# Frikallo/parakeet.cpp

Measured on NVIDIA H100. Metric: audio-seconds/sec (RTFx) tdt-ctc-110m 10s clips, higher is better.
Workload: dtype bf16x3

## Files before the change

### parakeet.cpp_b200/csrc/gemm_tc.cu

```cuda
#include <cuda.h>

#include "kernels.h"
#include "tc_prims.cuh"

namespace pk {
namespace {

using namespace tc;

constexpr int TC_THREADS = 384;
constexpr int CONSUMER_WARPS = 8;

template <int BN, int NPASS, bool LN = false>
struct TcCfg {
    static constexpr int A_BYTES = BM * BK * 2;
    static constexpr int W_BYTES = BN * BK * 2;
    static constexpr int PLANES = (NPASS == 3) ? 2 : 1;
    static constexpr int STAGE_BYTES = PLANES * (A_BYTES + W_BYTES);
    static constexpr int STAT_BYTES = LN ? 4 * BM * 4 * 4 : 0;
    static constexpr int AVAIL = 227 * 1024 - STAT_BYTES - 1024 - 256;
    static constexpr int STAGES = AVAIL / STAGE_BYTES > 8 ? 8 : AVAIL / STAGE_BYTES;
    static constexpr size_t SMEM = (size_t)STAGES * STAGE_BYTES + STAT_BYTES + 1024  + 256 ;
    static_assert(STAGES >= 2, "pipeline depth");
};

constexpr int LN_CL = 4;

template <int BN, int EK>
__device__ __forceinline__ void epilogue_regs(const float (&d)[BN / 2], const EpiParams &epi_param, int row0, int n0, int M, int N, int lane) {
    const EpiParams epi = epi_param;
    const int q = lane & 3;
    const int row = row0 + (lane >> 2) + ((q & 1) ? 8 : 0);
    const bool vec_ok = ((epi.ldo & 3) == 0) && ((N & 3) == 0);
    constexpr int G = 4;
#pragma unroll
    for (int j0 = 0; j0 < BN / 8; j0 += G) {
        float4 b[G], r[G];
#pragma unroll
        for (int g = 0; g < G; ++g) {
            const int col = n0 + 8 * (j0 + g) + 4 * (q >> 1);
            b[g] = r[g] = make_float4(0.f, 0.f, 0.f, 0.f);
            if (row < M && vec_ok && col + 4 <= N) {
                if (epi.bias) b[g] = __ldg(reinterpret_cast<const float4 *>(epi.bias + col));
                if (EK == EPI_RESID_F32) r[g] = *reinterpret_cast<const float4 *>(epi.resid + (size_t)row * epi.ldo + col);
            }
        }
#pragma unroll
        for (int g = 0; g < G; ++g) {
            const int j = j0 + g;
            const float s0 = (q & 1) ? d[4 * j] : d[4 * j + 2], s1 = (q & 1) ? d[4 * j + 1] : d[4 * j + 3];
            const float r0 = __shfl_xor_sync(0xffffffffu, s0, 1), r1 = __shfl_xor_sync(0xffffffffu, s1, 1);
            if (row >= M) continue;
            float4 v = (q & 1) ? make_float4(r0, r1, d[4 * j + 2], d[4 * j + 3]) : make_float4(d[4 * j], d[4 * j + 1], r0, r1);
            const int col = n0 + 8 * j + 4 * (q >> 1);
            if (vec_ok && col + 4 <= N) epi_store<EK>(epi, row, col, epi_math<EK>(v, b[g], r[g], epi.alpha));
            else epilogue4(epi_param, row, col, N, v);
        }
    }
}

template <int N>
__device__ __forceinline__ void fence_operands(float (&d)[N]) {
#pragma unroll
    for (int i = 0; i < N; ++i) asm volatile("" : "+f"(d[i])::"memory");
}

__device__ __forceinline__ float cluster_row_sum(float part, float *buf, int lrow, bool writer, uint32_t rank) {
    if (writer) {
        const uint32_t a = smem_u32(buf + lrow * LN_CL + rank);
#pragma unroll
        for (uint32_t r = 0; r < (uint32_t)LN_CL; ++r) st_cluster_f32(mapa_rank(a, r), part);
    }
    cluster_sync();
    const float4 v = *reinterpret_cast<const float4 *>(buf + lrow * LN_CL);
    return ((v.x + v.y) + v.z) + v.w;
}

__device__ __forceinline__ void epilogue_ln(const float (&d)[64], const LnEpi &ep, int row0, int lrow0, int n0, int M, int N, int lane,
                                            float *stat, uint32_t rank) {
    const int q = lane & 3;
    const int row = row0 + (lane >> 2) + ((q & 1) ? 8 : 0), lrow = lrow0 + (lane >> 2) + ((q & 1) ? 8 : 0);
    const bool writer = (q >> 1) == 0, live = row < M;
    float x[64];
#pragma unroll
    for (int j = 0; j < 16; ++j) {
        const float s0 = (q & 1) ? d[4 * j] : d[4 * j + 2], s1 = (q & 1) ? d[4 * j + 1] : d[4 * j + 3];
        const float r0 = __shfl_xor_sync(0xffffffffu, s0, 1), r1 = __shfl_xor_sync(0xffffffffu, s1, 1);
        const float4 v = (q & 1) ? make_float4(r0, r1, d[4 * j + 2], d[4 * j + 3]) : make_float4(d[4 * j], d[4 * j + 1], r0, r1);
        const int col = n0 + 8 * j + 4 * (q >> 1);
        float4 b = make_float4(0.f, 0.f, 0.f, 0.f), r = b;
        if (ep.bias) b = __ldg(reinterpret_cast<const float4 *>(ep.bias + col));
        if (ep.resid && live) r = *reinterpret_cast<const float4 *>(ep.resid + (size_t)row * N + col);
        x[4 * j] = r.x + ep.alpha * (v.x + b.x);
        x[4 * j + 1] = r.y + ep.alpha * (v.y + b.y);
        x[4 * j + 2] = r.z + ep.alpha * (v.z + b.z);
        x[4 * j + 3] = r.w + ep.alpha * (v.w + b.w);
    }
    auto store_f32 = [&]() {
        if (!live || !ep.out_f32) return;
#pragma unroll
        for (int j = 0; j < 16; ++j)
            *reinterpret_cast<float4 *>(ep.out_f32 + (size_t)row * N + n0 + 8 * j + 4 * (q >> 1)) =
                make_float4(x[4 * j], x[4 * j + 1], x[4 * j + 2], x[4 * j + 3]);
    };
    auto layernorm = [&](const float *w, const float *bb, float *buf) {
        float s = 0.f;
#pragma unroll
        for (int i = 0; i < 64; ++i) s += x[i];
        s += __shfl_xor_sync(0xffffffffu, s, 2);
        const float mean = cluster_row_sum(s, buf, lrow, writer, rank) / (float)N;
        float c = 0.f;
#pragma unroll
        for (int i = 0; i < 64; ++i) c += (x[i] - mean) * (x[i] - mean);
        c += __shfl_xor_sync(0xffffffffu, c, 2);
        const float rstd = rsqrtf(cluster_row_sum(c, buf + BM * LN_CL, lrow, writer, rank) / (float)N + ep.eps);
#pragma unroll
        for (int j = 0; j < 16; ++j) {
            const int col = n0 + 8 * j + 4 * (q >> 1);
            const float4 g = __ldg(reinterpret_cast<const float4 *>(w + col)), o = __ldg(reinterpret_cast<const float4 *>(bb + col));
            x[4 * j] = (x[4 * j] - mean) * rstd * g.x + o.x;
            x[4 * j + 1] = (x[4 * j + 1] - mean) * rstd * g.y + o.y;
            x[4 * j + 2] = (x[4 * j + 2] - mean) * rstd * g.z + o.z;
            x[4 * j + 3] = (x[4 * j + 3] - mean) * rstd * g.w + o.w;
        }
    };
    if (!ep.out_ln1) store_f32();
    layernorm(ep.ln1_w, ep.ln1_b, stat);
    if (ep.out_ln1) store_f32();
    if (ep.ln2_w) layernorm(ep.ln2_w, ep.ln2_b, stat + 2 * BM * LN_CL);
    if (live) {
#pragma unroll
        for (int j = 0; j < 16; ++j)
            store_act4(ep.planes, (size_t)row * N + n0 + 8 * j + 4 * (q >> 1), make_float4(x[4 * j], x[4 * j + 1], x[4 * j + 2], x[4 * j + 3]));
    }
}

template <int BN, int NPASS, int EK, int CL, bool MC, bool LN>
__device__ __forceinline__ void gemm_tc_body(const CUtensorMap &tmA_hi, const CUtensorMap &tmA_lo, const CUtensorMap &tmW_hi,
                                             const CUtensorMap &tmW_lo, int M, int N, int K, const EpiParams &epi, const LnEpi &lnp) {
    using C = TcCfg<BN, NPASS, LN>;
    extern __shared__ uint8_t smem_raw[];
    uint8_t *tiles = reinterpret_cast<uint8_t *>((reinterpret_cast<uintptr_t>(smem_raw) + 1023) & ~(uintptr_t)1023);
    float *stat = reinterpret_cast<float *>(tiles + (size_t)C::STAGES * C::STAGE_BYTES);
    uint64_t *full = reinterpret_cast<uint64_t *>(tiles + (size_t)C::STAGES * C::STAGE_BYTES + C::STAT_BYTES), *empty = full + C::STAGES;

    const int warp = threadIdx.x >> 5, lane = threadIdx.x & 31, wg = threadIdx.x >> 7;
    const int nkb = K / BK;
    const int tiles_n = (N + BN - 1) / BN, tiles_m = (M + BM - 1) / BM;
    const uint32_t rank = CL > 1 ? cluster_ctarank() : 0u;
    const int group_n = tiles_n / CL, num_units = group_n * tiles_m;
    const int first = (int)blockIdx.x / CL, step = (int)gridDim.x / CL;

    if (threadIdx.x == 0) {
        for (int s = 0; s < C::STAGES; ++s) {
            mbar_init(&full[s], 1);
            mbar_init(&empty[s], CONSUMER_WARPS * (MC ? CL : 1));
        }
        asm volatile("fence.mbarrier_init.release.cluster;" ::: "memory");
    }
    if (CL > 1) cluster_sync();
    else __syncthreads();
    pdl_wait();
    pdl_trigger();

    if (wg == 0) {
        if (warp == 0 && elect_one()) {
            uint32_t it = 0;
            for (int u = first; u < num_units; u += step) {
                const int m0 = (u / group_n) * BM, n0 = ((u % group_n) * CL + (int)rank) * BN;
                for (int kb = 0; kb < nkb; ++kb, ++it) {
                    const int s = it % C::STAGES;
                    const uint32_t ph = (it / C::STAGES) & 1;
                    mbar_wait(&empty[s], ph ^ 1);
                    uint8_t *st = tiles + (size_t)s * C::STAGE_BYTES;
                    mbar_expect_tx(&full[s], C::STAGE_BYTES);
                    if (MC) {
                        constexpr int SL = BM / CL, SLB = SL * BK * 2;
                        constexpr uint16_t mask = (uint16_t)((1u << CL) - 1u);
                        tma_load_2d_mcast(st + rank * SLB, &tmA_hi, &full[s], kb * BK, m0 + (int)rank * SL, mask);
                        if (NPASS == 3) tma_load_2d_mcast(st + C::A_BYTES + C::W_BYTES + rank * SLB, &tmA_lo, &full[s], kb * BK, m0 + (int)rank * SL, mask);
                    } else {
                        tma_load_2d(st, &tmA_hi, &full[s], kb * BK, m0);
                        if (NPASS == 3) tma_load_2d(st + C::A_BYTES + C::W_BYTES, &tmA_lo, &full[s], kb * BK, m0);
                    }
                    tma_load_2d(st + C::A_BYTES, &tmW_hi, &full[s], kb * BK, n0);
                    if (NPASS == 3) tma_load_2d(st + 2 * C::A_BYTES + C::W_BYTES, &tmW_lo, &full[s], kb * BK, n0);
                }
            }
            pdl_trigger_late();
        }
        __syncwarp();
        if (LN) {
            const int n_sync = lnp.ln2_w ? 4 : 2;
            for (int i = 0; i < n_sync; ++i) cluster_sync();
        }
    } else {
        const int cw = wg - 1;
        const uint32_t a_off = (uint32_t)cw * 64u * 128u;
        auto release = [&](int s) {
            __syncwarp();
            if (lane == 0) {
                if (MC) {
                    const uint32_t a = smem_u32(&empty[s]);
#pragma unroll
                    for (uint32_t r = 0; r < (uint32_t)CL; ++r) mbar_arrive_cluster(mapa_rank(a, r));
                } else {
                    mbar_arrive(&empty[s]);
                }
            }
        };
        uint32_t it = 0;
        for (int u = first; u < num_units; u += step) {
            const int m0 = (u / group_n) * BM, n0 = ((u % group_n) * CL + (int)rank) * BN;
            float d[BN / 2];
#pragma unroll
            for (int i = 0; i < BN / 2; ++i) d[i] = 0.f;
            fence_operands(d);
            int prev_s = -1;
            for (int kb = 0; kb < nkb; ++kb, ++it) {
                const int s = it % C::STAGES;
                const uint32_t ph = (it / C::STAGES) & 1;
                mbar_wait(&full[s], ph);
                const uint32_t st = smem_u32(tiles + (size_t)s * C::STAGE_BYTES);
                const uint64_t a_hi = wgmma_desc_sw128(st + a_off), w_hi = wgmma_desc_sw128(st + C::A_BYTES);
                const uint64_t a_lo = wgmma_desc_sw128(st + C::A_BYTES + C::W_BYTES + a_off);
                const uint64_t w_lo = wgmma_desc_sw128(st + 2 * C::A_BYTES + C::W_BYTES);
                wgmma_fence();
#pragma unroll
                for (int k = 0; k < BK / WGMMA_K; ++k) {
                    const uint64_t koff = (uint64_t)((k * WGMMA_K * 2) >> 4);
                    wgmma_bf16<BN>(d, a_hi + koff, w_hi + koff);
                    if (NPASS == 3) {
                        wgmma_bf16<BN>(d, a_hi + koff, w_lo + koff);
                        wgmma_bf16<BN>(d, a_lo + koff, w_hi + koff);
                    }
                }
                wgmma_commit();
                wgmma_wait<1>();
                if (prev_s >= 0) release(prev_s);
                prev_s = s;
            }
            wgmma_wait<0>();
            fence_operands(d);
            if (prev_s >= 0) release(prev_s);
            const int lrow0 = cw * 64 + (warp & 3) * 16;
            if constexpr (LN) epilogue_ln(d, lnp, m0 + lrow0, lrow0, n0, M, N, lane, stat, rank);
            else epilogue_regs<BN, EK>(d, epi, m0 + lrow0, n0, M, N, lane);
        }
    }
    if (CL > 1) cluster_sync();
}

constexpr uint32_t ORDER_BAR = 1;
constexpr uint32_t PRODUCER_REGS = 40, CONSUMER_REGS = 232;

template <int BN, int NPASS, int EK>
__global__ void __launch_bounds__(TC_THREADS, 1)
gemm_tc_kernel(const __grid_constant__ CUtensorMap tmA_hi, const __grid_constant__ CUtensorMap tmA_lo,
               const __grid_constant__ CUtensorMap tmW_hi, const __grid_constant__ CUtensorMap tmW_lo, int M, int N,
               int K, const __grid_constant__ EpiParams epi) {
    using C = TcCfg<BN, NPASS>;
    extern __shared__ uint8_t smem_raw[];
    uint8_t *tiles = reinterpret_cast<uint8_t *>((reinterpret_cast<uintptr_t>(smem_raw) + 1023) & ~(uintptr_t)1023);
    uint64_t *full = reinterpret_cast<uint64_t *>(tiles + (size_t)C::STAGES * C::STAGE_BYTES), *empty = full + C::STAGES;

    const int warp = threadIdx.x >> 5, lane = threadIdx.x & 31, wg = threadIdx.x >> 7;
    const int nkb = K / BK;
    const int tiles_n = (N + BN - 1) / BN, num_units = tiles_n * ((M + BM - 1) / BM);

    if (threadIdx.x == 0) {
        for (int s = 0; s < C::STAGES; ++s) {
            mbar_init(&full[s], 1);
            mbar_init(&empty[s], 4);
        }
        asm volatile("fence.mbarrier_init.release.cluster;" ::: "memory");
    }
    __syncthreads();
    pdl_wait();
    pdl_trigger();

    if (wg == 0) {
        setmaxnreg_dec<PRODUCER_REGS>();
        if (warp == 0 && elect_one()) {
            uint32_t it = 0;
            for (int u = blockIdx.x; u < num_units; u += gridDim.x) {
                const int m0 = (u / tiles_n) * BM, n0 = (u % tiles_n) * BN;
                for (int kb = 0; kb < nkb; ++kb, ++it) {
                    const int s = it % C::STAGES;
                    const uint32_t ph = (it / C::STAGES) & 1;
                    mbar_wait(&empty[s], ph ^ 1);
                    uint8_t *st = tiles + (size_t)s * C::STAGE_BYTES;
                    mbar_expect_tx(&full[s], C::STAGE_BYTES);
                    tma_load_2d(st, &tmA_hi, &full[s], kb * BK, m0);
                    if (NPASS == 3) tma_load_2d(st + C::A_BYTES + C::W_BYTES, &tmA_lo, &full[s], kb * BK, m0);
                    tma_load_2d(st + C::A_BYTES, &tmW_hi, &full[s], kb * BK, n0);
                    if (NPASS == 3) tma_load_2d(st + 2 * C::A_BYTES + C::W_BYTES, &tmW_lo, &full[s], kb * BK, n0);
                }
            }
            pdl_trigger_late();
        }
    } else {
        setmaxnreg_inc<CONSUMER_REGS>();
        const int cw = wg - 1;
        auto release = [&](int s) {
            __syncwarp();
            if (lane == 0) mbar_arrive(&empty[s]);
        };
        constexpr uint32_t HALF = 64u * 128u;
        uint32_t it = (uint32_t)(cw * nkb);
        for (int j = cw;; j += 2) {
            const int u = (int)blockIdx.x + j * (int)gridDim.x;
            if (u >= num_units) break;
            const int m0 = (u / tiles_n) * BM, n0 = (u % tiles_n) * BN;
            float d0[BN / 2], d1[BN / 2];
#pragma unroll
            for (int i = 0; i < BN / 2; ++i) d0[i] = d1[i] = 0.f;
            fence_operands(d0);
            fence_operands(d1);
            if (j > 0) bar_sync(ORDER_BAR + cw, 256);
            int prev_s = -1;
            for (int kb = 0; kb < nkb; ++kb, ++it) {
                const int s = it % C::STAGES;
                const uint32_t ph = (it / C::STAGES) & 1;
                mbar_wait(&full[s], ph);
                const uint32_t st = smem_u32(tiles + (size_t)s * C::STAGE_BYTES);
                const uint64_t a_hi = wgmma_desc_sw128(st), w_hi = wgmma_desc_sw128(st + C::A_BYTES);
                const uint64_t a_lo = wgmma_desc_sw128(st + C::A_BYTES + C::W_BYTES);
                const uint64_t w_lo = wgmma_desc_sw128(st + 2 * C::A_BYTES + C::W_BYTES);
                const uint64_t a_hi1 = wgmma_desc_sw128(st + HALF), a_lo1 = wgmma_desc_sw128(st + C::A_BYTES + C::W_BYTES + HALF);
                wgmma_fence();
#pragma unroll
                for (int k = 0; k < BK / WGMMA_K; ++k) {
                    const uint64_t koff = (uint64_t)((k * WGMMA_K * 2) >> 4);
                    wgmma_bf16<BN>(d0, a_hi + koff, w_hi + koff);
                    wgmma_bf16<BN>(d1, a_hi1 + koff, w_hi + koff);
                    if (NPASS == 3) {
                        wgmma_bf16<BN>(d0, a_hi + koff, w_lo + koff);
                        wgmma_bf16<BN>(d1, a_hi1 + koff, w_lo + koff);
                        wgmma_bf16<BN>(d0, a_lo + koff, w_hi + koff);
                        wgmma_bf16<BN>(d1, a_lo1 + koff, w_hi + koff);
                    }
                }
                wgmma_commit();
                wgmma_wait<1>();
                if (prev_s >= 0) release(prev_s);
                prev_s = s;
            }
            it += (uint32_t)nkb;
            if ((int)blockIdx.x + (j + 1) * (int)gridDim.x < num_units) bar_arrive(ORDER_BAR + (1 - cw), 256);
            wgmma_wait<0>();
            fence_operands(d0);
            fence_operands(d1);
            if (prev_s >= 0) release(prev_s);
            const int lrow0 = (warp & 3) * 16;
            epilogue_regs<BN, EK>(d0, epi, m0 + lrow0, n0, M, N, lane);
            epilogue_regs<BN, EK>(d1, epi, m0 + 64 + lrow0, n0, M, N, lane);
        }
    }
}

template <int NPASS, int EK, int CL>
__global__ void __cluster_dims__(CL, 1, 1) __launch_bounds__(TC_THREADS, 1)
gemm_tc_cl_kernel(const __grid_constant__ CUtensorMap tmA_hi, const __grid_constant__ CUtensorMap tmA_lo,
                  const __grid_constant__ CUtensorMap tmW_hi, const __grid_constant__ CUtensorMap tmW_lo, int M, int N,
                  int K, const __grid_constant__ EpiParams epi) {
    gemm_tc_body<128, NPASS, EK, CL, true, false>(tmA_hi, tmA_lo, tmW_hi, tmW_lo, M, N, K, epi, LnEpi());
}

template <int NPASS, bool MC>
__global__ void __cluster_dims__(LN_CL, 1, 1) __launch_bounds__(TC_THREADS, 1)
gemm_tc_ln_kernel(const __grid_constant__ CUtensorMap tmA_hi, const __grid_constant__ CUtensorMap tmA_lo,
                  const __grid_constant__ CUtensorMap tmW_hi, const __grid_constant__ CUtensorMap tmW_lo, int M, int N,
                  int K, const __grid_constant__ LnEpi lnp) {
    gemm_tc_body<128, NPASS, EPI_BIAS_F32, LN_CL, MC, true>(tmA_hi, tmA_lo, tmW_hi, tmW_lo, M, N, K, EpiParams(), lnp);
}

typedef CUresult (*EncodeTiledFn)(CUtensorMap *, CUtensorMapDataType, cuuint32_t, void *, const cuuint64_t *,
                                  const cuuint64_t *, const cuuint32_t *, const cuuint32_t *, CUtensorMapInterleave,
                                  CUtensorMapSwizzle, CUtensorMapL2promotion, CUtensorMapFloatOOBfill);

EncodeTiledFn encode_fn() {
    static EncodeTiledFn fn = nullptr;
    if (!fn) {
        void *p = nullptr;
        cudaDriverEntryPointQueryResult qr;
        if (cudaGetDriverEntryPoint("cuTensorMapEncodeTiled", &p, cudaEnableDefault, &qr) == cudaSuccess &&
            qr == cudaDriverEntryPointSuccess)
            fn = reinterpret_cast<EncodeTiledFn>(p);
    }
    return fn;
}

int num_sms_cur() {
    int dev = 0;
    cudaGetDevice(&dev);
    static int sms_of[64] = {};
    if (!sms_of[dev & 63]) cudaDeviceGetAttribute(&sms_of[dev & 63], cudaDevAttrMultiProcessorCount, dev);
    return sms_of[dev & 63];
}

template <int BN, int NPASS, int EK>
cudaError_t launch_k(const TcOperand &A, const TcOperand &W, int M, int N, int K, const EpiParams &epi, cudaStream_t st) {
    using C = TcCfg<BN, NPASS>;
    static PerDeviceFlag attr_flag;
    bool &attr = attr_flag.cur();
    if (!attr) {
        cudaError_t e = cudaFuncSetAttribute(gemm_tc_kernel<BN, NPASS, EK>, cudaFuncAttributeMaxDynamicSharedMemorySize, (int)C::SMEM);
        if (e != cudaSuccess) return e;
        attr = true;
    }
    const int num_sms = num_sms_cur();
    const int num_tiles = ((N + BN - 1) / BN) * ((M + BM - 1) / BM);
    dim3 grid(num_tiles < num_sms ? num_tiles : num_sms);
    const CUtensorMap &alo = (NPASS == 3) ? A.lo : A.hi, &wlo = (NPASS == 3) ? W.lo : W.hi;
    launch_pdl(gemm_tc_kernel<BN, NPASS, EK>, dim3(grid), dim3(TC_THREADS), C::SMEM, st, A.hi, alo, W.hi, wlo, M, N, K, epi);
    return cudaGetLastError();
}

template <int BN, int NPASS>
cudaError_t launch_t(const TcOperand &A, const TcOperand &W, int M, int N, int K, const EpiParams &epi, cudaStream_t st) {
    switch (epi.kind) {
    case EPI_BIAS_F32: return launch_k<BN, NPASS, EPI_BIAS_F32>(A, W, M, N, K, epi, st);
    case EPI_BIAS_RELU_F32: return launch_k<BN, NPASS, EPI_BIAS_RELU_F32>(A, W, M, N, K, epi, st);
    case EPI_BIAS_RELU_ACT: return launch_k<BN, NPASS, EPI_BIAS_RELU_ACT>(A, W, M, N, K, epi, st);
    case EPI_BIAS_SILU_ACT: return launch_k<BN, NPASS, EPI_BIAS_SILU_ACT>(A, W, M, N, K, epi, st);
    case EPI_RESID_F32: return launch_k<BN, NPASS, EPI_RESID_F32>(A, W, M, N, K, epi, st);
    case EPI_GLU_F32: return launch_k<BN, NPASS, EPI_GLU_F32>(A, W, M, N, K, epi, st);
    case EPI_BIAS_ACT: return launch_k<BN, NPASS, EPI_BIAS_ACT>(A, W, M, N, K, epi, st);
    case EPI_QKV_ACT: return launch_k<BN, NPASS, EPI_QKV_ACT>(A, W, M, N, K, epi, st);
    default: return cudaErrorInvalidValue;
    }
}

template <int NPASS, int EK, int CL>
cudaError_t launch_kcl(const TcOperand &A_sl, const TcOperand &W, int M, int N, int K, const EpiParams &epi, cudaStream_t st) {
    using C = TcCfg<128, NPASS>;
    static PerDeviceFlag attr_flag;
    static int max_clusters[64] = {};
    int dev = 0;
    cudaGetDevice(&dev);
    const int num_sms = num_sms_cur();
    if (!attr_flag.cur()) {
        cudaError_t e = cudaFuncSetAttribute(gemm_tc_cl_kernel<NPASS, EK, CL>, cudaFuncAttributeMaxDynamicSharedMemorySize, (int)C::SMEM);
        if (e != cudaSuccess) return e;
        cudaLaunchConfig_t q = {};
        q.gridDim = dim3((unsigned)(num_sms / CL * CL));
        q.blockDim = dim3(TC_THREADS);
        q.dynamicSmemBytes = C::SMEM;
        int mc = 0;
        if (cudaOccupancyMaxActiveClusters(&mc, gemm_tc_cl_kernel<NPASS, EK, CL>, &q) != cudaSuccess || mc < 1) {
            cudaGetLastError();
            mc = num_sms / CL;
        }
        max_clusters[dev & 63] = mc;
        attr_flag.cur() = true;
    }
    const int units = ((N / 128) / CL) * ((M + BM - 1) / BM);
    int ncl = max_clusters[dev & 63];
    if (ncl > num_sms / CL) ncl = num_sms / CL;
    if (ncl > units) ncl = units;
    const CUtensorMap &alo = (NPASS == 3) ? A_sl.lo : A_sl.hi, &wlo = (NPASS == 3) ? W.lo : W.hi;
    return launch_pdl(gemm_tc_cl_kernel<NPASS, EK, CL>, dim3((unsigned)(ncl * CL)), dim3(TC_THREADS), C::SMEM, st, A_sl.hi, alo, W.hi, wlo, M, N, K, epi);
}

template <int NPASS, bool MC>
cudaError_t launch_ln(const TcOperand &A, const TcOperand &W, int M, int N, int K, const LnEpi &ep, cudaStream_t st) {
    using C = TcCfg<128, NPASS, true>;
    static PerDeviceFlag attr_flag;
    if (!attr_flag.cur()) {
        cudaError_t e = cudaFuncSetAttribute(gemm_tc_ln_kernel<NPASS, MC>, cudaFuncAttributeMaxDynamicSharedMemorySize, (int)C::SMEM);
        if (e != cudaSuccess) return e;
        attr_flag.cur() = true;
    }
    const CUtensorMap &alo = (NPASS == 3) ? A.lo : A.hi, &wlo = (NPASS == 3) ? W.lo : W.hi;
    const int row_blocks = (M + BM - 1) / BM;
    return launch_pdl(gemm_tc_ln_kernel<NPASS, MC>, dim3((unsigned)(LN_CL * row_blocks)), dim3(TC_THREADS), C::SMEM, st, A.hi, alo, W.hi, wlo, M, N, K, ep);
}

}

bool make_tc_operand(TcOperand *out, const bf16 *hi, const bf16 *lo, uint64_t rows, uint64_t K, uint32_t box_rows) {
    EncodeTiledFn fn = encode_fn();
    if (!fn || !hi || (K % 8) != 0) return false;
    const cuuint64_t gdim[2] = {K, rows};
    const cuuint64_t gstr[1] = {K * sizeof(bf16)};
    const cuuint32_t box[2] = {(cuuint32_t)BK, box_rows};
    const cuuint32_t estr[2] = {1, 1};
    if (fn(&out->hi, CU_TENSOR_MAP_DATA_TYPE_BFLOAT16, 2, const_cast<bf16 *>(hi), gdim, gstr, box, estr,
           CU_TENSOR_MAP_INTERLEAVE_NONE, CU_TENSOR_MAP_SWIZZLE_128B, CU_TENSOR_MAP_L2_PROMOTION_L2_256B,
           CU_TENSOR_MAP_FLOAT_OOB_FILL_NONE) != CUDA_SUCCESS)
        return false;
    out->has_lo = lo != nullptr;
    if (lo && fn(&out->lo, CU_TENSOR_MAP_DATA_TYPE_BFLOAT16, 2, const_cast<bf16 *>(lo), gdim, gstr, box, estr,
                 CU_TENSOR_MAP_INTERLEAVE_NONE, CU_TENSOR_MAP_SWIZZLE_128B, CU_TENSOR_MAP_L2_PROMOTION_L2_256B,
                 CU_TENSOR_MAP_FLOAT_OOB_FILL_NONE) != CUDA_SUCCESS)
        return false;
    out->box_rows = box_rows;
    return true;
}

int tc_tile_n(int N) { return N <= 64 ? 64 : 128; }

bool gemm_tc_cluster_supported(int N, int epi_kind, int cl) {
    return (cl == 2 || cl == 4) && N % (128 * cl) == 0 && (epi_kind == EPI_BIAS_SILU_ACT || epi_kind == EPI_GLU_F32 || epi_kind == EPI_QKV_ACT);
}

cudaError_t launch_gemm_tc(const TcOperand &A, const TcOperand &W, int M, int N, int K, bool split3, const EpiParams &epi, cudaStream_t st,
                           int cl, const TcOperand *A_slice) {
    if (M <= 0 || N <= 0) return cudaSuccess;
    if (K % BK != 0 || A.box_rows != BM) return cudaErrorInvalidValue;
    if (split3 && !(A.has_lo && W.has_lo)) return cudaErrorInvalidValue;
    if (cl > 1 && split3 && A_slice && A_slice->has_lo && (int)A_slice->box_rows * cl == BM && W.box_rows == 128 && gemm_tc_cluster_supported(N, epi.kind, cl)) {
        switch (epi.kind) {
        case EPI_BIAS_SILU_ACT: return cl == 2 ? launch_kcl<3, EPI_BIAS_SILU_ACT, 2>(*A_slice, W, M, N, K, epi, st) : launch_kcl<3, EPI_BIAS_SILU_ACT, 4>(*A_slice, W, M, N, K, epi, st);
        case EPI_GLU_F32: return cl == 2 ? launch_kcl<3, EPI_GLU_F32, 2>(*A_slice, W, M, N, K, epi, st) : launch_kcl<3, EPI_GLU_F32, 4>(*A_slice, W, M, N, K, epi, st);
        default: return cl == 2 ? launch_kcl<3, EPI_QKV_ACT, 2>(*A_slice, W, M, N, K, epi, st) : launch_kcl<3, EPI_QKV_ACT, 4>(*A_slice, W, M, N, K, epi, st);
        }
    }
    if (W.box_rows == 128) return split3 ? launch_t<128, 3>(A, W, M, N, K, epi, st) : launch_t<128, 1>(A, W, M, N, K, epi, st);
    if (W.box_rows == 64) return split3 ? launch_t<64, 3>(A, W, M, N, K, epi, st) : launch_t<64, 1>(A, W, M, N, K, epi, st);
    return cudaErrorInvalidValue;
}

bool gemm_tc_ln_supported(int N) { return N == LN_CL * 128; }

cudaError_t launch_gemm_tc_ln(const TcOperand &A, const TcOperand &W, int M, int N, int K, bool split3, const LnEpi &epi, cudaStream_t st) {
    if (M <= 0) return cudaSuccess;
    if (!gemm_tc_ln_supported(N) || K % BK != 0 || W.box_rows != 128 || !epi.ln1_w || !epi.ln1_b) return cudaErrorInvalidValue;
    if (split3 && !(A.has_lo && W.has_lo)) return cudaErrorInvalidValue;
    if (A.box_rows == BM / LN_CL) return split3 ? launch_ln<3, true>(A, W, M, N, K, epi, st) : launch_ln<1, true>(A, W, M, N, K, epi, st);
    if (A.box_rows == BM) return split3 ? launch_ln<3, false>(A, W, M, N, K, epi, st) : launch_ln<1, false>(A, W, M, N, K, epi, st);
    return cudaErrorInvalidValue;
}

}
```

### parakeet.cpp_b200/csrc/tc_prims.cuh

```cuda
#pragma once
#include <cuda.h>

#include "kernels.h"

namespace pk {
namespace tc {

constexpr int BM = 128;
constexpr int BK = 64;
constexpr int WGMMA_K = 16;


__device__ __forceinline__ uint32_t smem_u32(const void *p) { return (uint32_t)__cvta_generic_to_shared(p); }

__device__ __forceinline__ void mbar_init(uint64_t *bar, uint32_t count) {
    asm volatile("mbarrier.init.shared::cta.b64 [%0], %1;" ::"r"(smem_u32(bar)), "r"(count));
}
__device__ __forceinline__ void mbar_expect_tx(uint64_t *bar, uint32_t bytes) {
    asm volatile("mbarrier.arrive.expect_tx.shared::cta.b64 _, [%0], %1;" ::"r"(smem_u32(bar)), "r"(bytes) : "memory");
}
__device__ __forceinline__ void mbar_wait(uint64_t *bar, uint32_t parity) {
    const uint32_t addr = smem_u32(bar);
    uint32_t done = 0;
    for (uint32_t spin = 0; !done; ++spin) {
        asm volatile(
            "{\n\t.reg .pred p;\n\t"
            "mbarrier.try_wait.parity.shared::cta.b64 p, [%1], %2;\n\t"
            "selp.u32 %0, 1, 0, p;\n\t}"
            : "=r"(done)
            : "r"(addr), "r"(parity)
            : "memory");
        if (spin > (1u << 26)) __trap();
    }
}
__device__ __forceinline__ void mbar_arrive(uint64_t *bar) {
    asm volatile("mbarrier.arrive.shared::cta.b64 _, [%0];" ::"r"(smem_u32(bar)) : "memory");
}
constexpr uint64_t L2_EVICT_LAST = 0x14F0000000000000ull;
__device__ __forceinline__ void tma_load_2d(void *smem_dst, const CUtensorMap *tm, uint64_t *bar, int c0, int c1, uint64_t policy = L2_EVICT_LAST) {
    asm volatile(
        "cp.async.bulk.tensor.2d.shared::cluster.global.mbarrier::complete_tx::bytes.L2::cache_hint [%0], [%1, {%3, %4}], [%2], %5;"
        ::"r"(smem_u32(smem_dst)), "l"(reinterpret_cast<uint64_t>(tm)), "r"(smem_u32(bar)), "r"(c0), "r"(c1), "l"(policy)
        : "memory");
}
__device__ __forceinline__ void tma_load_2d_mcast(void *smem_dst, const CUtensorMap *tm, uint64_t *bar, int c0, int c1, uint16_t cta_mask,
                                                  uint64_t policy = L2_EVICT_LAST) {
    asm volatile(
        "cp.async.bulk.tensor.2d.shared::cluster.global.mbarrier::complete_tx::bytes.multicast::cluster.L2::cache_hint [%0], [%1, {%4, %5}], [%2], %3, %6;"
        ::"r"(smem_u32(smem_dst)), "l"(reinterpret_cast<uint64_t>(tm)), "r"(smem_u32(bar)), "h"(cta_mask), "r"(c0), "r"(c1), "l"(policy)
        : "memory");
}
__device__ __forceinline__ uint32_t cluster_ctarank() {
    uint32_t r;
    asm volatile("mov.u32 %0, %%cluster_ctarank;" : "=r"(r));
    return r;
}
__device__ __forceinline__ void cluster_sync() {
    asm volatile("barrier.cluster.arrive.release.aligned;\n\tbarrier.cluster.wait.acquire.aligned;" ::: "memory");
}
__device__ __forceinline__ uint32_t mapa_rank(uint32_t saddr, uint32_t rank) {
    uint32_t r;
    asm volatile("mapa.shared::cluster.u32 %0, %1, %2;" : "=r"(r) : "r"(saddr), "r"(rank));
    return r;
}
__device__ __forceinline__ void mbar_arrive_cluster(uint32_t cluster_addr) {
    asm volatile("mbarrier.arrive.release.cluster.shared::cluster.b64 _, [%0];" ::"r"(cluster_addr) : "memory");
}
__device__ __forceinline__ void st_cluster_f32(uint32_t cluster_addr, float v) {
    asm volatile("st.shared::cluster.f32 [%0], %1;" ::"r"(cluster_addr), "f"(v) : "memory");
}

__device__ __forceinline__ bool elect_one() {
    uint32_t pred;
    asm volatile(
        "{\n\t.reg .pred p;\n\t"
        "elect.sync _|p, 0xffffffff;\n\t"
        "selp.u32 %0, 1, 0, p;\n\t}"
        : "=r"(pred));
    return pred != 0;
}

__device__ __forceinline__ uint64_t wgmma_desc_sw128(uint32_t saddr) {
    uint64_t d = 0;
    d |= (uint64_t)((saddr & 0x3FFFF) >> 4);
    d |= (uint64_t)1 << 16;
    d |= (uint64_t)(1024 >> 4) << 32;
    d |= (uint64_t)1 << 62;
    return d;
}
__device__ __forceinline__ void bar_sync(uint32_t id, uint32_t count) { asm volatile("bar.sync %0, %1;" ::"r"(id), "r"(count) : "memory"); }
__device__ __forceinline__ void bar_arrive(uint32_t id, uint32_t count) { asm volatile("bar.arrive %0, %1;" ::"r"(id), "r"(count) : "memory"); }

template <uint32_t R>
__device__ __forceinline__ void setmaxnreg_dec() { asm volatile("setmaxnreg.dec.sync.aligned.u32 %0;" ::"n"(R)); }
template <uint32_t R>
__device__ __forceinline__ void setmaxnreg_inc() { asm volatile("setmaxnreg.inc.sync.aligned.u32 %0;" ::"n"(R)); }

__device__ __forceinline__ void wgmma_fence() { asm volatile("wgmma.fence.sync.aligned;" ::: "memory"); }
__device__ __forceinline__ void wgmma_commit() { asm volatile("wgmma.commit_group.sync.aligned;" ::: "memory"); }
template <int N>
__device__ __forceinline__ void wgmma_wait() { asm volatile("wgmma.wait_group.sync.aligned %0;" ::"n"(N) : "memory"); }

template <int BN>
__device__ __forceinline__ void wgmma_bf16(float (&d)[BN / 2], uint64_t adesc, uint64_t bdesc);

template <>
__device__ __forceinline__ void wgmma_bf16<128>(float (&d)[64], uint64_t adesc, uint64_t bdesc) {
    asm volatile(
        "{\n\t.reg .pred p;\n\tsetp.ne.b32 p, 1, 0;\n\t"
        "wgmma.mma_async.sync.aligned.m64n128k16.f32.bf16.bf16 "
        "{%0, %1, %2, %3, %4, %5, %6, %7, %8, %9, %10, %11, %12, %13, %14, %15, "
        "%16, %17, %18, %19, %20, %21, %22, %23, %24, %25, %26, %27, %28, %29, %30, %31, "
        "%32, %33, %34, %35, %36, %37, %38, %39, %40, %41, %42, %43, %44, %45, %46, %47, "
        "%48, %49, %50, %51, %52, %53, %54, %55, %56, %57, %58, %59, %60, %61, %62, %63}, "
        "%64, %65, p, 1, 1, 0, 0;\n\t}"
        : "+f"(d[0]), "+f"(d[1]), "+f"(d[2]), "+f"(d[3]), "+f"(d[4]), "+f"(d[5]), "+f"(d[6]), "+f"(d[7]),
          "+f"(d[8]), "+f"(d[9]), "+f"(d[10]), "+f"(d[11]), "+f"(d[12]), "+f"(d[13]), "+f"(d[14]), "+f"(d[15]),
          "+f"(d[16]), "+f"(d[17]), "+f"(d[18]), "+f"(d[19]), "+f"(d[20]), "+f"(d[21]), "+f"(d[22]), "+f"(d[23]),
          "+f"(d[24]), "+f"(d[25]), "+f"(d[26]), "+f"(d[27]), "+f"(d[28]), "+f"(d[29]), "+f"(d[30]), "+f"(d[31]),
          "+f"(d[32]), "+f"(d[33]), "+f"(d[34]), "+f"(d[35]), "+f"(d[36]), "+f"(d[37]), "+f"(d[38]), "+f"(d[39]),
          "+f"(d[40]), "+f"(d[41]), "+f"(d[42]), "+f"(d[43]), "+f"(d[44]), "+f"(d[45]), "+f"(d[46]), "+f"(d[47]),
          "+f"(d[48]), "+f"(d[49]), "+f"(d[50]), "+f"(d[51]), "+f"(d[52]), "+f"(d[53]), "+f"(d[54]), "+f"(d[55]),
          "+f"(d[56]), "+f"(d[57]), "+f"(d[58]), "+f"(d[59]), "+f"(d[60]), "+f"(d[61]), "+f"(d[62]), "+f"(d[63])
        : "l"(adesc), "l"(bdesc));
}

template <>
__device__ __forceinline__ void wgmma_bf16<64>(float (&d)[32], uint64_t adesc, uint64_t bdesc) {
    asm volatile(
        "{\n\t.reg .pred p;\n\tsetp.ne.b32 p, 1, 0;\n\t"
        "wgmma.mma_async.sync.aligned.m64n64k16.f32.bf16.bf16 "
        "{%0, %1, %2, %3, %4, %5, %6, %7, %8, %9, %10, %11, %12, %13, %14, %15, "
        "%16, %17, %18, %19, %20, %21, %22, %23, %24, %25, %26, %27, %28, %29, %30, %31}, "
        "%32, %33, p, 1, 1, 0, 0;\n\t}"
        : "+f"(d[0]), "+f"(d[1]), "+f"(d[2]), "+f"(d[3]), "+f"(d[4]), "+f"(d[5]), "+f"(d[6]), "+f"(d[7]),
          "+f"(d[8]), "+f"(d[9]), "+f"(d[10]), "+f"(d[11]), "+f"(d[12]), "+f"(d[13]), "+f"(d[14]), "+f"(d[15]),
          "+f"(d[16]), "+f"(d[17]), "+f"(d[18]), "+f"(d[19]), "+f"(d[20]), "+f"(d[21]), "+f"(d[22]), "+f"(d[23]),
          "+f"(d[24]), "+f"(d[25]), "+f"(d[26]), "+f"(d[27]), "+f"(d[28]), "+f"(d[29]), "+f"(d[30]), "+f"(d[31])
        : "l"(adesc), "l"(bdesc));
}

}
}
```

Measured before the change: 31590.

## Stage GEMM epilogue through swizzled shared memory with TMA bulk stores

Adds a staged epilogue path in which consumer warpgroups write accumulator chunks into 128B-swizzled shared-memory buffers and issue TMA tensor stores, and prefetch residual tiles with TMA loads, instead of per-thread global stores. It is chosen at launch when tensor maps for the outputs can be encoded and falls back to the register epilogue otherwise. The aim is to coalesce the output writes and overlap them with the next tile's compute. The cost is 32KB of shared memory for epilogue buffers, which can reduce the number of pipeline stages, plus extra named-barrier synchronisation per chunk.

```diff
diff --git a/parakeet.cpp_b200/csrc/gemm_tc.cu b/parakeet.cpp_b200/csrc/gemm_tc.cu
--- a/parakeet.cpp_b200/csrc/gemm_tc.cu
+++ b/parakeet.cpp_b200/csrc/gemm_tc.cu
@@ -11,17 +11,22 @@
 constexpr int TC_THREADS = 384;
 constexpr int CONSUMER_WARPS = 8;
 
-template <int BN, int NPASS, bool LN = false>
+constexpr int CHUNK_ROWS = 64, CHUNK_BYTES = CHUNK_ROWS * 128;
+
+template <int BN, int NPASS, bool LN = false, bool STAGED = false>
 struct TcCfg {
     static constexpr int A_BYTES = BM * BK * 2;
     static constexpr int W_BYTES = BN * BK * 2;
     static constexpr int PLANES = (NPASS == 3) ? 2 : 1;
     static constexpr int STAGE_BYTES = PLANES * (A_BYTES + W_BYTES);
     static constexpr int STAT_BYTES = LN ? 4 * BM * 4 * 4 : 0;
-    static constexpr int AVAIL = 227 * 1024 - STAT_BYTES - 1024 - 256;
+    static constexpr int EPI_BYTES = STAGED ? 2 * 2 * CHUNK_BYTES : 0;
+    static constexpr int AVAIL = 227 * 1024 - STAT_BYTES - EPI_BYTES - 1024 - 256;
     static constexpr int STAGES = AVAIL / STAGE_BYTES > 8 ? 8 : AVAIL / STAGE_BYTES;
-    static constexpr size_t SMEM = (size_t)STAGES * STAGE_BYTES + STAT_BYTES + 1024  + 256 ;
+    static constexpr size_t SMEM = (size_t)STAGES * STAGE_BYTES + STAT_BYTES + EPI_BYTES + 1024  + 256 ;
     static_assert(STAGES >= 2, "pipeline depth");
+    static_assert(SMEM <= 227 * 1024, "shared memory per CTA");
+    static_assert((2 * STAGES + (STAGED ? 4 : 0)) * 8 <= 256, "barrier space");
 };
 
 constexpr int LN_CL = 4;
@@ -63,6 +68,216 @@
 __device__ __forceinline__ void fence_operands(float (&d)[N]) {
 #pragma unroll
     for (int i = 0; i < N; ++i) asm volatile("" : "+f"(d[i])::"memory");
+}
+
+struct EpiMaps {
+    CUtensorMap out, hi, lo, resid;
+};
+
+constexpr uint32_t EPI_BAR = 3;
+
+__device__ __forceinline__ void sts_f2(uint32_t a, float x, float y) { asm volatile("st.shared.v2.f32 [%0], {%1, %2};" ::"r"(a), "f"(x), "f"(y) : "memory"); }
+__device__ __forceinline__ void sts_f1(uint32_t a, float x) { asm volatile("st.shared.f32 [%0], %1;" ::"r"(a), "f"(x) : "memory"); }
+__device__ __forceinline__ void sts_b2(uint32_t a, __nv_bfloat162 h) { asm volatile("st.shared.b32 [%0], %1;" ::"r"(a), "r"(*reinterpret_cast<uint32_t *>(&h)) : "memory"); }
+__device__ __forceinline__ float2 lds_f2(uint32_t a) {
+    float2 v;
+    asm volatile("ld.shared.v2.f32 {%0, %1}, [%2];" : "=f"(v.x), "=f"(v.y) : "r"(a) : "memory");
+    return v;
+}
+
+struct Stager {
+    uint32_t buf;
+    uint32_t cnt;
+    __device__ __forceinline__ static bool leader() { return (threadIdx.x & 127) == 0; }
+    __device__ __forceinline__ static uint32_t b32() {
+        const uint32_t t = threadIdx.x & 127, rl = ((t >> 5) << 4) + ((t & 31) >> 2), q = t & 3;
+        return rl * 128u + ((((q >> 1) ^ rl) & 7u) << 4) + 8u * (q & 1u);
+    }
+    __device__ __forceinline__ static uint32_t b16() {
+        const uint32_t t = threadIdx.x & 127, rl = ((t >> 5) << 4) + ((t & 31) >> 2), q = t & 3;
+        return rl * 128u + ((rl & 7u) << 4) + 4u * q;
+    }
+    __device__ __forceinline__ uint32_t cur() const { return buf + (cnt & 1u) * CHUNK_BYTES; }
+    __device__ __forceinline__ uint32_t rbar(uint32_t b) const {
+        const uint32_t cw = (threadIdx.x >> 7) - 1;
+        return buf + (2u - cw) * 2u * CHUNK_BYTES + 16u * cw + 8u * b;
+    }
+    __device__ __forceinline__ void load(const CUtensorMap *tm, uint32_t ahead, int c0, int r0) const {
+        const uint32_t b = (cnt + ahead) & 1u;
+        asm volatile("mbarrier.arrive.expect_tx.shared::cta.b64 _, [%0], %1;" ::"r"(rbar(b)), "r"(CHUNK_BYTES) : "memory");
+        asm volatile(
+            "cp.async.bulk.tensor.2d.shared::cluster.global.mbarrier::complete_tx::bytes [%0], [%1, {%3, %4}], [%2];"
+            ::"r"(buf + b * CHUNK_BYTES), "l"(reinterpret_cast<uint64_t>(tm)), "r"(rbar(b)), "r"(c0), "r"(r0)
+            : "memory");
+    }
+    __device__ __forceinline__ void wait_loaded() const { mbar_wait(rbar(cnt & 1u), (cnt >> 1) & 1u); }
+    __device__ __forceinline__ void store(const CUtensorMap *tm, int c0, int r0) {
+        fence_proxy_async_smem();
+        if (leader()) bulk_wait_read<0>();
+        __syncwarp();
+        bar_sync(EPI_BAR + (threadIdx.x >> 7) - 1, 128);
+        if (leader()) {
+            tma_store_2d(tm, cur(), c0, r0);
+            bulk_commit();
+        }
+        __syncwarp();
+        ++cnt;
+    }
+    __device__ __forceinline__ uint32_t nxt() const { return buf + ((cnt + 1u) & 1u) * CHUNK_BYTES; }
+    __device__ __forceinline__ void drain() const {
+        if (leader()) bulk_wait_read<0>();
+        __syncwarp();
+        bar_sync(EPI_BAR + (threadIdx.x >> 7) - 1, 128);
+    }
+    __device__ __forceinline__ void store_pair(const CUtensorMap *tm0, const CUtensorMap *tm1, int c0, int r0) {
+        fence_proxy_async_smem();
+        __syncwarp();
+        bar_sync(EPI_BAR + (threadIdx.x >> 7) - 1, 128);
+        if (leader()) {
+            tma_store_2d(tm0, cur(), c0, r0);
+            tma_store_2d(tm1, nxt(), c0, r0);
+            bulk_commit();
+        }
+        __syncwarp();
+        cnt += 2;
+    }
+};
+
+template <int BN, int EK, int NJ>
+__device__ __forceinline__ void epi_chunk(float (&d)[BN / 2], int j0, const EpiParams &epi, int n0, int N) {
+    constexpr int MK = EK == EPI_RESID_F32 ? EPI_BIAS_F32 : EK;
+    const int q = threadIdx.x & 3;
+#pragma unroll
+    for (int jj = 0; jj < NJ; ++jj) {
+        const int j = j0 + jj, col = n0 + 8 * j + 2 * q;
+        float2 b = make_float2(0.f, 0.f);
+        if (epi.bias && col < N)
+            asm volatile("ld.global.nc.v2.f32 {%0, %1}, [%2];" : "=f"(b.x), "=f"(b.y) : "l"(epi.bias + col));
+        const float4 v = epi_math<MK>(make_float4(d[4 * j], d[4 * j + 1], d[4 * j + 2], d[4 * j + 3]), make_float4(b.x, b.y, b.x, b.y),
+                                      make_float4(0.f, 0.f, 0.f, 0.f), epi.alpha);
+        d[4 * j] = v.x; d[4 * j + 1] = v.y; d[4 * j + 2] = v.z; d[4 * j + 3] = v.w;
+    }
+}
+
+template <int BN>
+__device__ __forceinline__ void put_f32(const Stager &sg, const float (&d)[BN / 2], int j0) {
+    const uint32_t a = sg.cur() + Stager::b32();
+#pragma unroll
+    for (int jj = 0; jj < 4; ++jj) {
+        const int j = j0 + jj;
+        sts_f2(a ^ (32u * jj), d[4 * j], d[4 * j + 1]);
+        sts_f2((a ^ (32u * jj)) + 1024u, d[4 * j + 2], d[4 * j + 3]);
+    }
+}
+template <int BN, bool LO>
+__device__ __forceinline__ void put_bf16(const Stager &sg, const float (&d)[BN / 2], int j0) {
+    const uint32_t a = sg.cur() + Stager::b16(), al = sg.nxt() + Stager::b16();
+#pragma unroll
+    for (int jj = 0; jj < 8; ++jj) {
+        const int j = j0 + jj;
+        const __nv_bfloat162 h0 = __floats2bfloat162_rn(d[4 * j], d[4 * j + 1]), h1 = __floats2bfloat162_rn(d[4 * j + 2], d[4 * j + 3]);
+        sts_b2(a ^ (16u * jj), h0);
+        sts_b2((a ^ (16u * jj)) + 1024u, h1);
+        if (LO) {
+            const float2 f0 = __bfloat1622float2(h0), f1 = __bfloat1622float2(h1);
+            sts_b2(al ^ (16u * jj), __floats2bfloat162_rn(d[4 * j] - f0.x, d[4 * j + 1] - f0.y));
+            sts_b2((al ^ (16u * jj)) + 1024u, __floats2bfloat162_rn(d[4 * j + 2] - f1.x, d[4 * j + 3] - f1.y));
+        }
+    }
+}
+template <int BN>
+__device__ __forceinline__ void put_glu(const Stager &sg, const float (&d)[BN / 2], int j0) {
+    const uint32_t a = sg.cur() + Stager::b16();
+#pragma unroll
+    for (int jj = 0; jj < 8; ++jj) {
+        const int j = j0 + jj;
+        sts_f1(a ^ (16u * jj), d[4 * j]);
+        sts_f1((a ^ (16u * jj)) + 1024u, d[4 * j + 1]);
+    }
+}
+
+template <int BN>
+__device__ __forceinline__ void resid_chunk(const Stager &sg, const float (&d)[BN / 2], int j0, float alpha) {
+    const uint32_t a = sg.cur() + Stager::b32();
+#pragma unroll
+    for (int jj = 0; jj < 4; ++jj) {
+        const int j = j0 + jj;
+        const uint32_t p0 = a ^ (32u * jj), p1 = p0 + 1024u;
+        const float2 r0 = lds_f2(p0), r1 = lds_f2(p1);
+        sts_f2(p0, r0.x + alpha * d[4 * j], r0.y + alpha * d[4 * j + 1]);
+        sts_f2(p1, r1.x + alpha * d[4 * j + 2], r1.y + alpha * d[4 * j + 3]);
+    }
+}
+
+template <int BN, int EK>
+__device__ __forceinline__ void epilogue_staged(float (&d)[BN / 2], const EpiParams &epi, const EpiMaps &om, Stager &sg, int row0,
+                                                int n0, int N, int next_row) {
+    constexpr int NCH = BN / 32, NG = BN / 64;
+    auto store = [&](const CUtensorMap *tm, int c0, int r0) {
+        sg.store(tm, c0, r0);
+        fence_operands(d);
+    };
+    if constexpr (EK == EPI_RESID_F32) {
+#pragma unroll
+        for (int s = 0; s < NCH; ++s) {
+            const int c0 = n0 + 32 * s;
+            if (c0 >= N) break;
+            if (Stager::leader()) {
+                bulk_wait_read<0>();
+                if (s + 1 < NCH && c0 + 32 < N) sg.load(&om.resid, 1, c0 + 32, row0);
+                else if (next_row >= 0) sg.load(&om.resid, 1, n0, next_row);
+            }
+            __syncwarp();
+            epi_chunk<BN, EK, 4>(d, 4 * s, epi, n0, N);
+            sg.wait_loaded();
+            resid_chunk<BN>(sg, d, 4 * s, epi.alpha);
+            store(&om.out, c0, row0);
+        }
+    } else {
+#pragma unroll
+        for (int g = 0; g < NG; ++g) {
+            const int c0 = n0 + 64 * g;
+            if (c0 >= N) break;
+            epi_chunk<BN, EK, 8>(d, 8 * g, epi, n0, N);
+            if constexpr (EK == EPI_GLU_F32) {
+                put_glu<BN>(sg, d, 8 * g);
+                store(&om.out, c0 / 2, row0);
+            } else if (EK == EPI_BIAS_F32 || EK == EPI_BIAS_RELU_F32) {
+                put_f32<BN>(sg, d, 8 * g);
+                store(&om.out, c0, row0);
+                if (c0 + 32 < N) {
+                    put_f32<BN>(sg, d, 8 * g + 4);
+                    store(&om.out, c0 + 32, row0);
+                }
+            } else if (EK == EPI_QKV_ACT && c0 < epi.qcols) {
+                sg.drain();
+                put_f32<BN>(sg, d, 8 * g);
+                store(&om.out, c0, row0);
+                put_f32<BN>(sg, d, 8 * g + 4);
+                store(&om.out, c0 + 32, row0);
+            } else {
+                const int pc = c0 - (EK == EPI_QKV_ACT ? epi.qcols : 0);
+                sg.drain();
+                if (EK != EPI_QKV_ACT && epi.act.f32) {
+                    put_f32<BN>(sg, d, 8 * g);
+                    store(&om.out, pc, row0);
+                    if (pc + 32 < N) {
+                        put_f32<BN>(sg, d, 8 * g + 4);
+                        store(&om.out, pc + 32, row0);
+                    }
+                }
+                if (epi.act.hi && epi.act.lo) {
+                    if (EK != EPI_QKV_ACT && epi.act.f32) sg.drain();
+                    put_bf16<BN, true>(sg, d, 8 * g);
+                    sg.store_pair(&om.hi, &om.lo, pc, row0);
+                    fence_operands(d);
+                } else if (epi.act.hi) {
+                    put_bf16<BN, false>(sg, d, 8 * g);
+                    store(&om.hi, pc, row0);
+                }
+            }
+        }
+    }
 }
 
 __device__ __forceinline__ float cluster_row_sum(float part, float *buf, int lrow, bool writer, uint32_t rank) {
@@ -254,15 +469,17 @@
 constexpr uint32_t ORDER_BAR = 1;
 constexpr uint32_t PRODUCER_REGS = 40, CONSUMER_REGS = 232;
 
-template <int BN, int NPASS, int EK>
+template <int BN, int NPASS, int EK, bool STAGED>
 __global__ void __launch_bounds__(TC_THREADS, 1)
 gemm_tc_kernel(const __grid_constant__ CUtensorMap tmA_hi, const __grid_constant__ CUtensorMap tmA_lo,
                const __grid_constant__ CUtensorMap tmW_hi, const __grid_constant__ CUtensorMap tmW_lo, int M, int N,
-               int K, const __grid_constant__ EpiParams epi) {
-    using C = TcCfg<BN, NPASS>;
+               int K, const __grid_constant__ EpiParams epi, const __grid_constant__ EpiMaps om) {
+    using C = TcCfg<BN, NPASS, false, STAGED>;
     extern __shared__ uint8_t smem_raw[];
     uint8_t *tiles = reinterpret_cast<uint8_t *>((reinterpret_cast<uintptr_t>(smem_raw) + 1023) & ~(uintptr_t)1023);
-    uint64_t *full = reinterpret_cast<uint64_t *>(tiles + (size_t)C::STAGES * C::STAGE_BYTES), *empty = full + C::STAGES;
+    uint8_t *chunks = tiles + (size_t)C::STAGES * C::STAGE_BYTES;
+    uint64_t *rbar = reinterpret_cast<uint64_t *>(chunks + C::EPI_BYTES);
+    uint64_t *full = rbar + (STAGED ? 4 : 0), *empty = full + C::STAGES;
 
     const int warp = threadIdx.x >> 5, lane = threadIdx.x & 31, wg = threadIdx.x >> 7;
     const int nkb = K / BK;
@@ -273,6 +490,8 @@
             mbar_init(&full[s], 1);
             mbar_init(&empty[s], 4);
         }
+        if (STAGED)
+            for (int i = 0; i < 4; ++i) mbar_init(&rbar[i], 1);
         asm volatile("fence.mbarrier_init.release.cluster;" ::: "memory");
     }
     __syncthreads();
@@ -306,6 +525,7 @@
             __syncwarp();
             if (lane == 0) mbar_arrive(&empty[s]);
         };
+        Stager sg{smem_u32(chunks) + (uint32_t)cw * 2u * CHUNK_BYTES, 0u};
         constexpr uint32_t HALF = 64u * 128u;
         uint32_t it = (uint32_t)(cw * nkb);
         for (int j = cw;; j += 2) {
@@ -348,14 +568,30 @@
             }
             it += (uint32_t)nkb;
             if ((int)blockIdx.x + (j + 1) * (int)gridDim.x < num_units) bar_arrive(ORDER_BAR + (1 - cw), 256);
+            if (EK == EPI_RESID_F32 && STAGED) {
+                if (Stager::leader()) {
+                    bulk_wait_read<0>();
+                    sg.load(&om.resid, 0, n0, m0);
+                }
+                __syncwarp();
+            }
             wgmma_wait<0>();
             fence_operands(d0);
             fence_operands(d1);
             if (prev_s >= 0) release(prev_s);
             const int lrow0 = (warp & 3) * 16;
-            epilogue_regs<BN, EK>(d0, epi, m0 + lrow0, n0, M, N, lane);
-            epilogue_regs<BN, EK>(d1, epi, m0 + 64 + lrow0, n0, M, N, lane);
-        }
+            if constexpr (STAGED) {
+                const bool two = m0 + 64 < M;
+                epilogue_staged<BN, EK>(d0, epi, om, sg, m0, n0, N, two ? m0 + 64 : -1);
+                fence_operands(d1);
+                if (two) epilogue_staged<BN, EK>(d1, epi, om, sg, m0 + 64, n0, N, -1);
+            } else {
+                epilogue_regs<BN, EK>(d0, epi, m0 + lrow0, n0, M, N, lane);
+                epilogue_regs<BN, EK>(d1, epi, m0 + 64 + lrow0, n0, M, N, lane);
+            }
+        }
+        if constexpr (STAGED)
+            if (Stager::leader()) bulk_wait<0>();
     }
 }
 
@@ -399,13 +635,47 @@
     return sms_of[dev & 63];
 }
 
-template <int BN, int NPASS, int EK>
-cudaError_t launch_k(const TcOperand &A, const TcOperand &W, int M, int N, int K, const EpiParams &epi, cudaStream_t st) {
-    using C = TcCfg<BN, NPASS>;
+bool encode_out(CUtensorMap *m, const void *p, bool f32, uint64_t width, uint64_t rows, uint64_t ld) {
+    EncodeTiledFn fn = encode_fn();
+    const uint64_t esz = f32 ? 4 : 2;
+    if (!fn || !p || (reinterpret_cast<uintptr_t>(p) & 15) || (ld * esz) % 16 || width == 0) return false;
+    const cuuint64_t gdim[2] = {width, rows};
+    const cuuint64_t gstr[1] = {ld * esz};
+    const cuuint32_t box[2] = {(cuuint32_t)(128 / esz), (cuuint32_t)CHUNK_ROWS};
+    const cuuint32_t estr[2] = {1, 1};
+    return fn(m, f32 ? CU_TENSOR_MAP_DATA_TYPE_FLOAT32 : CU_TENSOR_MAP_DATA_TYPE_BFLOAT16, 2, const_cast<void *>(p), gdim, gstr, box, estr,
+              CU_TENSOR_MAP_INTERLEAVE_NONE, CU_TENSOR_MAP_SWIZZLE_128B, CU_TENSOR_MAP_L2_PROMOTION_NONE,
+              CU_TENSOR_MAP_FLOAT_OOB_FILL_NONE) == CUDA_SUCCESS;
+}
+
+bool staged_maps(EpiMaps *om, const EpiParams &e, int M, int N) {
+    if (N % 4 || e.ldo % 4) return false;
+    switch (e.kind) {
+    case EPI_BIAS_F32:
+    case EPI_BIAS_RELU_F32: return encode_out(&om->out, e.out_f32, true, N, M, e.ldo);
+    case EPI_RESID_F32: return encode_out(&om->out, e.out_f32, true, N, M, e.ldo) && encode_out(&om->resid, e.resid, true, N, M, e.ldo);
+    case EPI_GLU_F32: return encode_out(&om->out, e.out_f32, true, N / 2, M, e.ldo);
+    case EPI_QKV_ACT:
+        if (e.qcols <= 0 || e.qcols % 64 || e.qcols >= N || e.act.f32 || !e.act.hi) return false;
+        return encode_out(&om->out, e.out_f32, true, e.qcols, M, e.qcols) && encode_out(&om->hi, e.act.hi, false, N - e.qcols, M, e.ldo) &&
+               (!e.act.lo || encode_out(&om->lo, e.act.lo, false, N - e.qcols, M, e.ldo));
+    case EPI_BIAS_RELU_ACT:
+    case EPI_BIAS_SILU_ACT:
+    case EPI_BIAS_ACT:
+        if (!e.act.f32 && !e.act.hi) return false;
+        return (!e.act.f32 || encode_out(&om->out, e.act.f32, true, N, M, e.ldo)) && (!e.act.hi || encode_out(&om->hi, e.act.hi, false, N, M, e.ldo)) &&
+               (!e.act.lo || encode_out(&om->lo, e.act.lo, false, N, M, e.ldo));
+    default: return false;
+    }
+}
+
+template <int BN, int NPASS, int EK, bool STAGED>
+cudaError_t launch_k(const TcOperand &A, const TcOperand &W, int M, int N, int K, const EpiParams &epi, const EpiMaps &om, cudaStream_t st) {
+    using C = TcCfg<BN, NPASS, false, STAGED>;
     static PerDeviceFlag attr_flag;
     bool &attr = attr_flag.cur();
     if (!attr) {
-        cudaError_t e = cudaFuncSetAttribute(gemm_tc_kernel<BN, NPASS, EK>, cudaFuncAttributeMaxDynamicSharedMemorySize, (int)C::SMEM);
+        cudaError_t e = cudaFuncSetAttribute(gemm_tc_kernel<BN, NPASS, EK, STAGED>, cudaFuncAttributeMaxDynamicSharedMemorySize, (int)C::SMEM);
         if (e != cudaSuccess) return e;
         attr = true;
     }
@@ -413,21 +683,28 @@
     const int num_tiles = ((N + BN - 1) / BN) * ((M + BM - 1) / BM);
     dim3 grid(num_tiles < num_sms ? num_tiles : num_sms);
     const CUtensorMap &alo = (NPASS == 3) ? A.lo : A.hi, &wlo = (NPASS == 3) ? W.lo : W.hi;
-    launch_pdl(gemm_tc_kernel<BN, NPASS, EK>, dim3(grid), dim3(TC_THREADS), C::SMEM, st, A.hi, alo, W.hi, wlo, M, N, K, epi);
+    launch_pdl(gemm_tc_kernel<BN, NPASS, EK, STAGED>, dim3(grid), dim3(TC_THREADS), C::SMEM, st, A.hi, alo, W.hi, wlo, M, N, K, epi, om);
     return cudaGetLastError();
+}
+
+template <int BN, int NPASS, int EK>
+cudaError_t launch_e(const TcOperand &A, const TcOperand &W, int M, int N, int K, const EpiParams &epi, cudaStream_t st) {
+    EpiMaps om = {};
+    if (staged_maps(&om, epi, M, N)) return launch_k<BN, NPASS, EK, true>(A, W, M, N, K, epi, om, st);
+    return launch_k<BN, NPASS, EK, false>(A, W, M, N, K, epi, om, st);
 }
 
 template <int BN, int NPASS>
 cudaError_t launch_t(const TcOperand &A, const TcOperand &W, int M, int N, int K, const EpiParams &epi, cudaStream_t st) {
     switch (epi.kind) {
-    case EPI_BIAS_F32: return launch_k<BN, NPASS, EPI_BIAS_F32>(A, W, M, N, K, epi, st);
-    case EPI_BIAS_RELU_F32: return launch_k<BN, NPASS, EPI_BIAS_RELU_F32>(A, W, M, N, K, epi, st);
-    case EPI_BIAS_RELU_ACT: return launch_k<BN, NPASS, EPI_BIAS_RELU_ACT>(A, W, M, N, K, epi, st);
-    case EPI_BIAS_SILU_ACT: return launch_k<BN, NPASS, EPI_BIAS_SILU_ACT>(A, W, M, N, K, epi, st);
-    case EPI_RESID_F32: return launch_k<BN, NPASS, EPI_RESID_F32>(A, W, M, N, K, epi, st);
-    case EPI_GLU_F32: return launch_k<BN, NPASS, EPI_GLU_F32>(A, W, M, N, K, epi, st);
-    case EPI_BIAS_ACT: return launch_k<BN, NPASS, EPI_BIAS_ACT>(A, W, M, N, K, epi, st);
-    case EPI_QKV_ACT: return launch_k<BN, NPASS, EPI_QKV_ACT>(A, W, M, N, K, epi, st);
+    case EPI_BIAS_F32: return launch_e<BN, NPASS, EPI_BIAS_F32>(A, W, M, N, K, epi, st);
+    case EPI_BIAS_RELU_F32: return launch_e<BN, NPASS, EPI_BIAS_RELU_F32>(A, W, M, N, K, epi, st);
+    case EPI_BIAS_RELU_ACT: return launch_e<BN, NPASS, EPI_BIAS_RELU_ACT>(A, W, M, N, K, epi, st);
+    case EPI_BIAS_SILU_ACT: return launch_e<BN, NPASS, EPI_BIAS_SILU_ACT>(A, W, M, N, K, epi, st);
+    case EPI_RESID_F32: return launch_e<BN, NPASS, EPI_RESID_F32>(A, W, M, N, K, epi, st);
+    case EPI_GLU_F32: return launch_e<BN, NPASS, EPI_GLU_F32>(A, W, M, N, K, epi, st);
+    case EPI_BIAS_ACT: return launch_e<BN, NPASS, EPI_BIAS_ACT>(A, W, M, N, K, epi, st);
+    case EPI_QKV_ACT: return launch_e<BN, NPASS, EPI_QKV_ACT>(A, W, M, N, K, epi, st);
     default: return cudaErrorInvalidValue;
     }
 }
diff --git a/parakeet.cpp_b200/csrc/tc_prims.cuh b/parakeet.cpp_b200/csrc/tc_prims.cuh
--- a/parakeet.cpp_b200/csrc/tc_prims.cuh
+++ b/parakeet.cpp_b200/csrc/tc_prims.cuh
@@ -19,8 +19,7 @@
 __device__ __forceinline__ void mbar_expect_tx(uint64_t *bar, uint32_t bytes) {
     asm volatile("mbarrier.arrive.expect_tx.shared::cta.b64 _, [%0], %1;" ::"r"(smem_u32(bar)), "r"(bytes) : "memory");
 }
-__device__ __forceinline__ void mbar_wait(uint64_t *bar, uint32_t parity) {
-    const uint32_t addr = smem_u32(bar);
+__device__ __forceinline__ void mbar_wait(uint32_t addr, uint32_t parity) {
     uint32_t done = 0;
     for (uint32_t spin = 0; !done; ++spin) {
         asm volatile(
@@ -33,6 +32,7 @@
         if (spin > (1u << 26)) __trap();
     }
 }
+__device__ __forceinline__ void mbar_wait(uint64_t *bar, uint32_t parity) { mbar_wait(smem_u32(bar), parity); }
 __device__ __forceinline__ void mbar_arrive(uint64_t *bar) {
     asm volatile("mbarrier.arrive.shared::cta.b64 _, [%0];" ::"r"(smem_u32(bar)) : "memory");
 }
@@ -50,6 +50,18 @@
         ::"r"(smem_u32(smem_dst)), "l"(reinterpret_cast<uint64_t>(tm)), "r"(smem_u32(bar)), "h"(cta_mask), "r"(c0), "r"(c1), "l"(policy)
         : "memory");
 }
+__device__ __forceinline__ void tma_store_2d(const CUtensorMap *tm, uint32_t smem_src, int c0, int c1) {
+    asm volatile("cp.async.bulk.tensor.2d.global.shared::cta.bulk_group [%0, {%2, %3}], [%1];"
+                 ::"l"(reinterpret_cast<uint64_t>(tm)), "r"(smem_src), "r"(c0), "r"(c1)
+                 : "memory");
+}
+__device__ __forceinline__ void bulk_commit() { asm volatile("cp.async.bulk.commit_group;" ::: "memory"); }
+template <int N>
+__device__ __forceinline__ void bulk_wait_read() { asm volatile("cp.async.bulk.wait_group.read %0;" ::"n"(N) : "memory"); }
+template <int N>
+__device__ __forceinline__ void bulk_wait() { asm volatile("cp.async.bulk.wait_group %0;" ::"n"(N) : "memory"); }
+__device__ __forceinline__ void fence_proxy_async_smem() { asm volatile("fence.proxy.async.shared::cta;" ::: "memory"); }
+
 __device__ __forceinline__ uint32_t cluster_ctarank() {
     uint32_t r;
     asm volatile("mov.u32 %0, %%cluster_ctarank;" : "=r"(r));
```

Result: faster. 35540, median of 6 (+12.5%).
